# vsahni3/cross-attention-ViT

Measured on AMD Instinct MI355X. Metric: 3D patch-tokens/sec fwd+bwd, 2-modality 128^3 p16 ViT, higher is better.
Workload: dtype bf16; 1 GPU; configs[1]: ModelCross d=768 H=12 mlp=3072 2x2 blocks, 2 modalities, 128^3 volume, 16^3 patches (N=513), dropout 0; per_gpu_batch=126, global_batch=126, seq_len=513, parallelism=dp1, step=zero-grad + weight bf16 cast + fwd + loss + bwd, optimizer_step=excluded, launch=eager (one launch per kernel)

## Files before the change

cross-attention-vit_amd/csrc/gemm.hip:

```cpp
#include "xvit_common.h"

#include <atomic>
#include <mutex>
#include <algorithm>
#include <string>

namespace xvit {

struct GemmParams {
  const bf16* A; const bf16* B; void* C; const float* bias; const float* res; bf16* aux;
  int64_t lda, ldb, ldc, ldr, ldaux;
  int64_t sA, sB, sC, sBias, sR, sAux;
  int M, N, K, k_per_split, split_k, ntm, ntn;
  int c_f32, act, accumulate;
  int res_row_mod, res_row_off, seg_rows, seg_skip, row_off;
  float* slab;
  float* colsum;
  float drop_p, drop_inv; uint64_t drop_seed;
  const uint64_t* drop_epoch;
  int aux_deriv;
  int narrow_epi;
  int ncg;
  struct PatchGather {
    int mode;
// ... 285 lines not shown
      }
    }
  }
  if (csum && !part) {
#pragma unroll
    for (int e = 0; e < 4; ++e) {
      float t = cs4[e];
      t += __shfl_xor(t, 16);
      t += __shfl_xor(t, 32);
      cs4[e] = t;
    }
    if (lane < 16 && col < p.N) {
#pragma unroll
      for (int e = 0; e < 4; ++e) unsafeAtomicAdd(csum + col + e, cs4[e]);
    }
  }
}

constexpr int TBM = 256, TBN = 256;
constexpr int T_OPER = TBM * BK * 2;
constexpr int T_STAGE = 2 * T_OPER;
constexpr int T_LDS = 2 * T_STAGE;

__device__ __forceinline__ int gather_krow_token(const GemmParams::PatchGather& g, int kr) {
  const int nw = 64 / g.Dn;
  if (nw & 1) return kr;
  const int a = kr >> 1, b = kr & 1, wa = a / g.Dn, d = a - wa * g.Dn;
  return d + g.Dn * (2 * wa + b);
}

template <bool KS>
struct BigLoader {
  __amdgpu_buffer_rsrc_t rsrc;
  uint32_t voff[4];
  uint32_t kstep;
  __device__ __forceinline__ void init(const bf16* tile_base, int64_t bytes_avail, int64_t ld, int wave, int lane, const GemmParams::PatchGather* perm = nullptr) {
    rsrc = make_rsrc(tile_base, clamp_bytes(bytes_avail));
#pragma unroll
    for (int j = 0; j < 4; ++j) {
      const int piece = wave * 4 + j;
      if (KS) {
        const int krow = piece * 2 + (lane >> 5);
        const int chunk = (lane & 31) ^ swz_ks(krow);
        const int srow = perm ? gather_krow_token(*perm, krow) : krow;
        voff[j] = (uint32_t)(srow * ld * 2 + chunk * 16);
      } else {
        const int row = piece * 8 + (lane >> 3);
        const int chunk = (lane & 7) ^ swz_kc(row);
        voff[j] = (uint32_t)(row * ld * 2 + chunk * 16);
      }
    }
    kstep = KS ? (uint32_t)(BK * ld * 2) : (uint32_t)(BK * 2);
  }
  __device__ __forceinline__ void init_gather_rows(const GemmParams::PatchGather& g, const bf16* vol, int m0, int M, int wave, int lane) {
    rsrc = make_rsrc(vol, g.vol_bytes);
#pragma unroll
    for (int j = 0; j < 4; ++j) {
      const int ii = lane >> 3, rl = (wave * 4 + j) * 8 + ii, row = m0 + wave * 32 + (ii & 3) * 8 + 2 * j + (ii >> 2);
      const int chunk = (lane & 7) ^ swz_kc(rl);
      const int smp = row / g.ntok, n = row - smp * g.ntok;
      voff[j] = (row < M && n >= g.cls) ? 2u * (gather_sample_origin(g, smp) + gather_patch_origin(g, n - g.cls) + gather_elem_off(g, chunk * 8)) : GATHER_OOB;
    }
    kstep = 0;
  }
  __device__ __forceinline__ void init_gather_ks(const GemmParams::PatchGather& g, const bf16* vol, int n0, int N, int wave, int lane) {
    rsrc = make_rsrc(vol, g.vol_bytes);
#pragma unroll
    for (int j = 0; j < 4; ++j) {
      const int krow = (wave * 4 + j) * 2 + (lane >> 5);
      const int e = n0 + (((lane & 31) ^ swz_ks(krow)) << 3);
      const int tok = gather_krow_token(g, krow);
      voff[j] = e < N ? 2u * ((uint32_t)((tok % g.Dn) * g.dp * g.Sz + (tok / g.Dn) * g.wp) + gather_elem_off(g, e)) : GATHER_OOB;
    }
    kstep = 0;
  }
  __device__ __forceinline__ void place_tokens(const GemmParams::PatchGather& g, int ktg, uint32_t total, int64_t ld, bool volume, const uint32_t (&fixed)[4], int wave, int lane) {
#pragma unroll
    for (int j = 0; j < 4; ++j) {
      const int krow = (wave * 4 + j) * 2 + (lane >> 5);
      const GatherTok t = gather_token(g, (uint32_t)ktg * 64u + (uint32_t)krow, total);
      voff[j] = !t.ok || fixed[j] == GATHER_OOB ? GATHER_OOB : (volume ? 2u * t.vol + fixed[j] : t.row * (uint32_t)(ld * 2) + fixed[j]);
    }
  }
  __device__ __forceinline__ void issue_at(XVIT_LDS char* image, int wave, uint32_t soff) const {
#pragma unroll
    for (int j = 0; j < 4; ++j) glds16(rsrc, image + (wave * 4 + j) * 1024, voff[j], soff);
  }
  __device__ __forceinline__ void issue(XVIT_LDS char* image, int wave, int kt) const { issue_at(image, wave, (uint32_t)kt * kstep); }
};

__device__ __forceinline__ uint32_t gather_soff_rows(const GemmParams::PatchGather& g, int ktg) { return 2u * gather_elem_off(g, ktg * 64); }
struct GatherStep { uint32_t a, b; };
__device__ __forceinline__ GatherStep gather_soff_wgrad(const GemmParams::PatchGather& g, int ktg, int64_t lda) {
  const int spk = g.pcount >> 6, smp = ktg / spk, r = ktg - smp * spk;
  const int wsteps = (g.Dn * g.Wn) >> 6, h = r / wsteps, wpart = (r - h * wsteps) * (64 / g.Dn);
  GatherStep o;
  o.a = (uint32_t)(((int64_t)smp * g.ntok + g.cls + r * 64) * lda * 2);
  o.b = 2u * (gather_sample_origin(g, smp) + (uint32_t)(h * g.hp * g.Sy + wpart * g.wp));
  return o;
}

typedef __attribute__((__vector_size__(4 * sizeof(unsigned)))) unsigned u32x4_dbg;
template <bool KS, int NT_>
struct BigFrag {
  uint32_t off[KS ? 2 * NT_ : 2];
  __device__ __forceinline__ void init(int first, int lane) {
    if (KS) {
      const int g = lane >> 4, i = lane & 15, q = i >> 2, p = i & 3;
#pragma unroll
      for (int t = 0; t < NT_; ++t)
#pragma unroll
        for (int s = 0; s < 2; ++s) {
          const int krow = 8 * g + 4 * s + q;
          const int ch = (first + t) * 2 + (p >> 1);
          off[t * 2 + s] = (uint32_t)(512 * krow + 16 * (ch ^ swz_ks(krow)) + 8 * (p & 1));
        }
    } else {
      const int row = first * 16 + (lane & 15);
#pragma unroll
      for (int kk = 0; kk < 2; ++kk) off[kk] = (uint32_t)(row * 128 + (((kk * 4 + (lane >> 4)) ^ swz_kc(row)) << 4));
    }
  }
  __device__ __forceinline__ bf16x8 read(const XVIT_LDS char* image, int t, int kk) const {
#ifdef XVIT_DEBUG_NO_LDSREAD
    u32x4_dbg v = {off[0] * 2654435761u, off[0] * 40503u + 12345u, (uint32_t)t * 0x9E3779B9u ^ off[0], 0x3F803F80u ^ (off[0] << 3)};
    v &= 0xBFFFBFFFu;
    asm volatile("" : "+v"(v));
    return __builtin_bit_cast(bf16x8, v);
#endif
    if (KS) {
      const s16x4 lo = lds_read_tr16(image + off[t * 2 + 0] + kk * 32 * 512);
      const s16x4 hi = lds_read_tr16(image + off[t * 2 + 1] + kk * 32 * 512);
      s16x8 v = {lo[0], lo[1], lo[2], lo[3], hi[0], hi[1], hi[2], hi[3]};
      return __builtin_bit_cast(bf16x8, v);
    } else {
      return *(const XVIT_LDS bf16x8*)(image + off[kk] + t * 16 * 128);
    }
  }
};

template <int S, int PF, int NA, int NB>
__device__ __forceinline__ void mma_sched_steps() {
  constexpr int reads = (S + PF < 16 ? NA : 0) + (S >= 4 && S < 8 ? NB : 0);
  if constexpr (reads > 0) __builtin_amdgcn_sched_group_barrier(0x100, reads, 0);
  __builtin_amdgcn_sched_group_barrier(0x008, 4, 0);
  if constexpr (S + 1 < 16) mma_sched_steps<S + 1, PF, NA, NB>();
}

template <bool A_KS, bool B_KS>
__device__ __forceinline__ void big_tile_mma(const XVIT_LDS char* sa, const XVIT_LDS char* sb, const BigFrag<A_KS, 8>& fa, const BigFrag<B_KS, 4>& fb,
                                             f32x4 (&acc)[8][4], const BigLoader<A_KS>& la, const BigLoader<B_KS>& lb, __amdgpu_buffer_rsrc_t ra,
                                             __amdgpu_buffer_rsrc_t rb, XVIT_LDS char* nxt, int wave, uint32_t soff_a, uint32_t soff_b) {
  constexpr int PF = 2;
  constexpr int NA = A_KS ? 2 : 1, NB = B_KS ? 2 : 1;
  bf16x8 b0[4], b1[4], a[16];
#pragma unroll
  for (int t = 0; t < 4; ++t) b0[t] = fb.read(sb, t, 0);
#pragma unroll
  for (int s = 0; s < PF; ++s) a[s] = fa.read(sa, s & 7, s >> 3);
#pragma unroll
  for (int s = 0; s < 16; ++s) {
#ifndef XVIT_DEBUG_NO_DMA
    if (s < 4) glds16(ra, nxt + (wave * 4 + s) * 1024, la.voff[s], soff_a);
    else if (s < 8) glds16(rb, nxt + T_OPER + (wave * 4 + s - 4) * 1024, lb.voff[s - 4], soff_b);
#endif
    if (s + PF < 16) a[s + PF] = fa.read(sa, (s + PF) & 7, (s + PF) >> 3);
    if (s >= 4 && s < 8) b1[s - 4] = fb.read(sb, s - 4, 1);
#pragma unroll
    for (int j = 0; j < 4; ++j)
      acc[s & 7][j] = __builtin_amdgcn_mfma_f32_16x16x32_bf16(s < 8 ? b0[j] : b1[j], a[s], acc[s & 7][j], 0, 0, 0);
  }
  __builtin_amdgcn_sched_group_barrier(0x100, 4 * NB + PF * NA, 0);
  mma_sched_steps<0, PF, NA, NB>();
}

#ifndef XVIT_EPI_STORE_AUX
#define XVIT_EPI_STORE_AUX 2
#endif
#ifndef XVIT_EPI_LOAD_AUX
#define XVIT_EPI_LOAD_AUX 2
#endif
#ifndef XVIT_EPI_RES_AUX
#define XVIT_EPI_RES_AUX 2
#endif
typedef __attribute__((__vector_size__(2 * sizeof(unsigned)))) unsigned u32x2_t;
typedef __attribute__((__vector_size__(4 * sizeof(unsigned)))) unsigned u32x4_t;
constexpr uint32_t OOB = 0xFFFFFFF0u;
constexpr int EPI_WAVE_BYTES = 64 * 256;

struct BigEpi {
  __amdgpu_buffer_rsrc_t rc, raux, rres, rslab;
  bool has_res, has_aux, to_slab;
  uint32_t col;
  bool col_ok;
  f32x4 bias;
  f32x4 csum;
  float* colsum_dst;
  uint64_t drop_base;
  uint32_t row, c, aux, res, slab;
  uint32_t rrem, rmod, srem, smod;
  uint32_t c_step, aux_step, res_step, slab_step, c_gap, res_wrap;
};

struct LoadCursor { uint32_t row, aux; };
struct EpiLoads { u32x2_t aux[4]; };

// ... 187 lines not shown
  for (int b = 0; b < 2; ++b) {
    const int it = (R & 3) * 2 + b;
    const f32x4 v0 = *(const XVIT_LDS f32x4*)(slice + it * 2048 + roffw[it & 1][0]);
    const f32x4 v1 = *(const XVIT_LDS f32x4*)(slice + it * 2048 + roffw[it & 1][1]);
    wide_body<ACT, DROP>(p, e, v0, v1, cur.aux[b]);
  }
  __builtin_amdgcn_sched_barrier(0);
  if constexpr (R < 7) wide_regions<ACT, DROP, R + 1>(p, e, lc, nxt, acc, slice, woff, roffw);
}

template <int ACT, bool DROP>
__device__ __forceinline__ void wide_epilogue(const GemmParams& p, WideEpi& e, const f32x4 (&acc)[8][4], XVIT_LDS char* slice, const uint32_t (&woff)[4],
                                              const uint32_t (&roffw)[2][2], float* colsum_dst) {
  WideCursor lc = {e.row, e.aux};
  WideLoads first;
  if constexpr (ACT == XVIT_ACT_DGELU || ACT == ACT_MULAUX) wide_issue_aux(p, e, lc, first);
  wide_regions<ACT, DROP, 0>(p, e, lc, first, acc, slice, woff, roffw);
  if (colsum_dst) {
#pragma unroll
    for (int c = 0; c < 4; ++c) {
      float t0 = e.csum0[c], t1 = e.csum1[c];
#pragma unroll
      for (int o = 8; o < 64; o <<= 1) { t0 += __shfl_xor(t0, o); t1 += __shfl_xor(t1, o); }
      e.csum0[c] = t0; e.csum1[c] = t1;
    }
    if ((threadIdx.x & 63) < 8 && e.col_ok) {
#pragma unroll
      for (int c = 0; c < 4; ++c) { unsafeAtomicAdd(colsum_dst + c, e.csum0[c]); unsafeAtomicAdd(colsum_dst + 4 + c, e.csum1[c]); }
    }
  }
}

template <int ACT>
__device__ __forceinline__ void wave_tile_epilogue_wide(const GemmParams& p, const f32x4 (&acc)[8][4], XVIT_LDS char* smem, int wave, int lane, int row0, int col0,
                                                        int batch) {
  WideEpi e;
  e.rc = make_rsrc((const char*)p.C + batch * p.sC * 2, clamp_bytes(0x7FFFFFF0ll));
  e.has_aux = p.aux != nullptr;
  const bool has_bias = p.bias != nullptr;
  e.raux = make_rsrc(e.has_aux ? (const void*)(p.aux + batch * p.sAux) : (const void*)p.C, e.has_aux ? 0x7FFFFFF0u : 0u);
  const __amdgpu_buffer_rsrc_t rbias = make_rsrc(has_bias ? (const void*)(p.bias + batch * p.sBias) : (const void*)p.C, has_bias ? (uint32_t)(p.N * 4) : 0u);
  int pin = 0;
  asm volatile("" : "+v"(pin));
  const int wl = lane + pin;
  uint32_t woff[4], roffw[2][2];
  {
    const int r = wl & 15, g = wl >> 4, c = wl & 7, rr = wl >> 3;
#pragma unroll
    for (int j = 0; j < 4; ++j) woff[j] = (uint32_t)(r * 256 + (((j * 4 + g) ^ r) << 4));
#pragma unroll
    for (int par = 0; par < 2; ++par)
#pragma unroll
      for (int k = 0; k < 2; ++k) roffw[par][k] = (uint32_t)(rr * 256 + (((2 * c + k) ^ ((par * 8 + rr) & 15)) << 4));
  }
  XVIT_LDS char* slice = smem + wave * EPI_WAVE_BYTES;
  e.col = (uint32_t)(col0 + (wl & 7) * 8);
  e.col_ok = e.col < (uint32_t)p.N;
  e.bias0 = __builtin_bit_cast(f32x4, __builtin_amdgcn_raw_buffer_load_b128(rbias, e.col * 4, 0, 0));
  e.bias1 = __builtin_bit_cast(f32x4, __builtin_amdgcn_raw_buffer_load_b128(rbias, e.col * 4 + 16, 0, 0));
  e.drop_base = (uint64_t)batch * ((uint64_t)p.M * p.N);
  e.csum0 = f32x4{0.f, 0.f, 0.f, 0.f}; e.csum1 = f32x4{0.f, 0.f, 0.f, 0.f};
  float* colsum_dst = p.colsum ? p.colsum + batch * p.sBias + e.col : nullptr;
  e.row = (uint32_t)(row0 + (wl >> 3));
  e.c = e.row * (uint32_t)p.ldc * 2u + e.col * 2u;
  e.aux = e.row * (uint32_t)p.ldaux * 2u + e.col * 2u;
  e.c_step = 8u * (uint32_t)p.ldc * 2u;
  e.aux_step = 8u * (uint32_t)p.ldaux * 2u;
  wide_epilogue<ACT, false>(p, e, acc, slice, woff, roffw, colsum_dst);
}

template <bool PERM = false>
__device__ __forceinline__ void wave_tile_epilogue(const GemmParams& p, const f32x4 (&acc)[8][4], XVIT_LDS char* smem, int wave, int lane, int row0, int col0,
                                                   int batch, int split) {
  const int nbatch = gridDim.z / p.split_k;
  BigEpi e;
  const int64_t celt = p.c_f32 ? 4 : 2;
  e.rc = make_rsrc((const char*)p.C + batch * p.sC * celt, clamp_bytes(0x7FFFFFF0ll));
  e.has_aux = p.aux != nullptr; e.has_res = p.res != nullptr; e.to_slab = p.slab != nullptr;
  const bool has_bias = p.bias != nullptr;
  e.raux = make_rsrc(e.has_aux ? (const void*)(p.aux + batch * p.sAux) : (const void*)p.C, e.has_aux ? 0x7FFFFFF0u : 0u);
  e.rres = make_rsrc(e.has_res ? (const void*)(p.res + batch * p.sR) : (const void*)p.C, e.has_res ? 0x7FFFFFF0u : 0u);
  const __amdgpu_buffer_rsrc_t rbias = make_rsrc(has_bias ? (const void*)(p.bias + batch * p.sBias) : (const void*)p.C, has_bias ? (uint32_t)(p.N * 4) : 0u);
  e.rslab = make_rsrc(e.to_slab ? (const void*)(p.slab + ((int64_t)split * nbatch + batch) * (int64_t)p.M * p.N) : (const void*)p.C,
                      e.to_slab ? clamp_bytes((int64_t)p.M * p.N * 4) : 0u);
  int pin = 0;
  asm volatile("" : "+v"(pin));
  const int wl = lane + pin;
  uint32_t woff[8], roff[4];
  {
    const int r = wl & 15, g = wl >> 4, k = wl & 15, rr = wl >> 4;
#pragma unroll
    for (int j = 0; j < 4; ++j) woff[j] = woff[4 + j] = (uint32_t)(r * 256 + (((j * 4 + g) ^ r) << 4));
    if constexpr (PERM) {
#pragma unroll
      for (int half = 0; half < 2; ++half) {
        const int l32 = 16 * half + r, jj = l32 >> 3, ii = l32 & 7, rho = (ii & 3) * 8 + 2 * jj + (ii >> 2);
#pragma unroll
        for (int j = 0; j < 4; ++j) woff[half * 4 + j] = (uint32_t)(rho * 256 + (((j * 4 + g) ^ (rho & 15)) << 4));
      }
    }
#pragma unroll
    for (int q = 0; q < 4; ++q) roff[q] = (uint32_t)(rr * 256 + ((k ^ (q * 4 + rr)) << 4));
  }
  XVIT_LDS char* slice = smem + wave * EPI_WAVE_BYTES;
  e.col = (uint32_t)(col0 + (wl & 15) * 4);
  e.col_ok = e.col < (uint32_t)p.N;
  e.bias = __builtin_bit_cast(f32x4, __builtin_amdgcn_raw_buffer_load_b128(rbias, e.col * 4, 0, 0));
  e.drop_base = (uint64_t)batch * ((uint64_t)p.M * p.N);
  e.csum = f32x4{0.f, 0.f, 0.f, 0.f};
  e.colsum_dst = p.colsum ? p.colsum + batch * p.sBias + e.col : nullptr;
  e.row = (uint32_t)(row0 + (wl >> 4));
  {
    const bool rmap = p.res_row_mod > 0, smap = p.seg_rows > 0;
    e.rmod = rmap ? (uint32_t)p.res_row_mod : 0x7FFFFFFFu;
    e.smod = smap ? (uint32_t)p.seg_rows : 0x7FFFFFFFu;
    e.rrem = rmap ? e.row % e.rmod : e.row;
    e.srem = smap ? e.row % e.smod : e.row;
    const uint32_t rrow = rmap ? (uint32_t)p.res_row_off + e.rrem : e.row;
    const uint32_t orow = smap ? e.row + (e.row / e.smod) * (uint32_t)p.seg_skip + (uint32_t)p.row_off : e.row;
    const uint32_t ce = p.c_f32 ? 4u : 2u;
    e.c = orow * (uint32_t)p.ldc * ce + e.col * ce;
    e.aux = e.row * (uint32_t)p.ldaux * 2u + e.col * 2u;
    e.res = rrow * (uint32_t)p.ldr * 4u + e.col * 4u;
    e.slab = e.row * (uint32_t)p.N * 4u + e.col * 4u;
    e.c_step = 4u * (uint32_t)p.ldc * ce;
    e.aux_step = 4u * (uint32_t)p.ldaux * 2u;
    e.res_step = 4u * (uint32_t)p.ldr * 4u;
    e.slab_step = 4u * (uint32_t)p.N * 4u;
    e.c_gap = smap ? (uint32_t)p.seg_skip * (uint32_t)p.ldc * ce : 0u;
    e.res_wrap = rmap ? e.rmod * (uint32_t)p.ldr * 4u : 0u;
  }
  if constexpr (PERM) {
    big_epilogue<XVIT_ACT_NONE, false, true>(p, e, acc, slice, woff, roff);
    return;
  }
  if (p.drop_p > 0.f) {
    if (p.act == XVIT_ACT_GELU) big_epilogue<XVIT_ACT_GELU, true>(p, e, acc, slice, woff, roff);
    else if (p.act == XVIT_ACT_DGELU) big_epilogue<XVIT_ACT_DGELU, true>(p, e, acc, slice, woff, roff);
    else big_epilogue<XVIT_ACT_NONE, true>(p, e, acc, slice, woff, roff);
  } else if (p.act == XVIT_ACT_GELU) big_epilogue<XVIT_ACT_GELU, false>(p, e, acc, slice, woff, roff);
  else if (p.act == XVIT_ACT_DGELU) big_epilogue<XVIT_ACT_DGELU, false>(p, e, acc, slice, woff, roff);
  else big_epilogue<XVIT_ACT_NONE, false>(p, e, acc, slice, woff, roff);
}

#ifdef XVIT_GEMM_CLOCK_PROBE
__device__ long long xvit_dbg_clk[2 * 4096];
struct ClockProbe {
  long long c0, w0;
  __device__ ClockProbe() : c0(clock64()), w0(wall_clock64()) {}
  __device__ ~ClockProbe() {
    if (threadIdx.x == 0 && blockIdx.z == 0 && blockIdx.x < 4096) { xvit_dbg_clk[2 * blockIdx.x] = clock64() - c0; xvit_dbg_clk[2 * blockIdx.x + 1] = wall_clock64() - w0; }
  }
};
#endif
template <bool A_KS, bool B_KS, int WIDE_ACT, int GATHER = 0>
__global__ __launch_bounds__(512, 2) void gemm_big_kernel(const GemmParams p) {
  extern __shared__ __attribute__((aligned(16))) char smem_raw[];
  XVIT_LDS char* smem = (XVIT_LDS char*)smem_raw;
#ifdef XVIT_GEMM_CLOCK_PROBE
  ClockProbe clock_probe;
#endif
  const int tid = threadIdx.x, lane = tid & 63, wave = uniform(tid >> 6);
  const int wr = wave >> 2, wc = wave & 3;

  const int nblk = gridDim.x, total = nblk * gridDim.z, lin = blockIdx.x + nblk * blockIdx.z;
  const int q8 = total >> 3, r8 = total & 7, xcd = lin & 7;
  const int logical = (xcd < r8 ? xcd * (q8 + 1) : r8 * (q8 + 1) + (xcd - r8) * q8) + (lin >> 3);
  const int zz = logical / nblk, tile = logical - zz * nblk;
  const int grp = min(tile / (p.ntm * p.ncg), (p.ntn - 1) / p.ncg);
  const int rem = tile - grp * p.ntm * p.ncg;
  const int gw = min(p.ncg, p.ntn - grp * p.ncg);
  const int tm = rem / gw, tn = grp * p.ncg + (rem - tm * gw);
  const int m0 = tm * TBM, n0 = tn * TBN;
  const int batch = zz / p.split_k, split = zz - batch * p.split_k;
  const int k_begin = split * p.k_per_split;
  const int k_end = min(p.K, k_begin + p.k_per_split);
  const int nk = (k_end - k_begin + BK - 1) / BK;

  BigLoader<A_KS> la;
  BigLoader<B_KS> lb;
  {
    const bf16* Ab = p.A + batch * p.sA;
    if constexpr (GATHER == 1) la.init_gather_rows(p.g, Ab, m0, p.M, wave, lane);
    else if constexpr (GATHER == 2 || GATHER == 3) {
      const int64_t rows = (int64_t)(p.K / p.g.pcount) * p.g.ntok;
      la.init(Ab + m0, ((rows - 1) * p.lda + (p.M - m0)) * 2, p.lda, wave, lane, GATHER == 2 ? &p.g : nullptr);
    } else if (A_KS) la.init(Ab + (int64_t)k_begin * p.lda + m0, ((int64_t)(k_end - 1 - k_begin) * p.lda + (p.M - m0)) * 2, p.lda, wave, lane);
    else la.init(Ab + (int64_t)m0 * p.lda + k_begin, ((int64_t)(p.M - 1 - m0) * p.lda + (k_end - k_begin)) * 2, p.lda, wave, lane);
    const bf16* Bb = p.B + batch * p.sB;
    if constexpr (GATHER == 2 || GATHER == 3) lb.init_gather_ks(p.g, Bb, n0, p.N, wave, lane);
    else if (B_KS) lb.init(Bb + (int64_t)k_begin * p.ldb + n0, ((int64_t)(k_end - 1 - k_begin) * p.ldb + (p.N - n0)) * 2, p.ldb, wave, lane);
    else lb.init(Bb + (int64_t)n0 * p.ldb + k_begin, ((int64_t)(p.N - 1 - n0) * p.ldb + (k_end - k_begin)) * 2, p.ldb, wave, lane);
  }
  const int ktg0 = k_begin / BK;
  uint32_t fix_a[4], fix_b[4];
  if constexpr (GATHER == 3) {
#pragma unroll
    for (int j = 0; j < 4; ++j) {
      const int krow = (wave * 4 + j) * 2 + (lane >> 5);
      const int chunk = (lane & 31) ^ swz_ks(krow);
      fix_a[j] = m0 + chunk * 8 < p.M ? (uint32_t)(chunk * 16) : GATHER_OOB;
      const int e = n0 + (chunk << 3);
      fix_b[j] = e < p.N ? 2u * gather_elem_off(p.g, e) : GATHER_OOB;
    }
  }
  auto step_off = [&](int kt, uint32_t& oa, uint32_t& ob) {
    if constexpr (GATHER == 1) { oa = gather_soff_rows(p.g, ktg0 + kt); ob = (uint32_t)kt * lb.kstep; }
    else if constexpr (GATHER == 2) { GatherStep o; o = gather_soff_wgrad(p.g, ktg0 + kt, p.lda); oa = o.a; ob = o.b; }
    else if constexpr (GATHER == 3) {
      la.place_tokens(p.g, ktg0 + kt, (uint32_t)p.K, p.lda, false, fix_a, wave, lane);
      lb.place_tokens(p.g, ktg0 + kt, (uint32_t)p.K, 0, true, fix_b, wave, lane);
      oa = ob = 0u;
    }
    else { oa = (uint32_t)kt * la.kstep; ob = (uint32_t)kt * lb.kstep; }
  };
  BigFrag<A_KS, 8> fa;
  BigFrag<B_KS, 4> fb;
  fa.init(wr * 8, lane);
  fb.init(wc * 4, lane);

  f32x4 acc[8][4];
#pragma unroll
  for (int i = 0; i < 8; ++i)
#pragma unroll
    for (int j = 0; j < 4; ++j) acc[i][j] = f32x4{0.f, 0.f, 0.f, 0.f};

  const __amdgpu_buffer_rsrc_t null_rsrc = make_rsrc(p.A, 0u);
  if (nk > 0) {
    uint32_t oa, ob;
    step_off(0, oa, ob);
    la.issue_at(smem, wave, oa);
    lb.issue_at(smem + T_OPER, wave, ob);
  }
  for (int kt = 0; kt < nk; ++kt) {
    asm volatile("s_waitcnt vmcnt(0)" ::: "memory");
    __syncthreads();
    const bool more = kt + 1 < nk;
    uint32_t soff_a, soff_b;
    step_off(kt + 1, soff_a, soff_b);
    XVIT_LDS char* nxt = smem + ((kt + 1) & 1) * T_STAGE;
    const XVIT_LDS char* sa = smem + (kt & 1) * T_STAGE;
    const XVIT_LDS char* sb = sa + T_OPER;
#ifndef XVIT_DEBUG_NO_MMA
    big_tile_mma<A_KS, B_KS>(sa, sb, fa, fb, acc, la, lb, more ? la.rsrc : null_rsrc, more ? lb.rsrc : null_rsrc, nxt, wave, soff_a, soff_b);
#endif
  }

  asm volatile("s_waitcnt vmcnt(0)" ::: "memory");
  __syncthreads();
  if constexpr (WIDE_ACT >= 0) wave_tile_epilogue_wide<WIDE_ACT>(p, acc, smem, wave, lane, m0 + wr * 128, n0 + wc * 64, batch);
  else wave_tile_epilogue<GATHER == 1>(p, acc, smem, wave, lane, m0 + wr * 128, n0 + wc * 64, batch, split);
}

__global__ void splitk_epilogue_kernel(const GemmParams p, int nbatch) {
  const int nv = p.N >> 2;
  const int64_t per = (int64_t)p.M * nv, total = per * nbatch;
  for (int64_t i = (int64_t)blockIdx.x * blockDim.x + threadIdx.x; i < total; i += (int64_t)gridDim.x * blockDim.x) {
    const int b = (int)(i / per);
    const int64_t r = i - (int64_t)b * per;
    const int row = (int)(r / nv), col = (int)(r - (int64_t)row * nv) * 4;
    f32x4 v = {0.f, 0.f, 0.f, 0.f};
    for (int s = 0; s < p.split_k; ++s) v += *(const f32x4*)(p.slab + (((int64_t)s * nbatch + b) * p.M + row) * p.N + col);
    const f32x4 o = epilogue_apply_rt(p, v, row, col, b * p.sC, p.bias ? p.bias + b * p.sBias : nullptr, p.res ? p.res + b * p.sR : nullptr,
                                      p.aux ? p.aux + b * p.sAux : nullptr);
    if (p.colsum) {
#pragma unroll
      for (int e = 0; e < 4; ++e) unsafeAtomicAdd(p.colsum + b * p.sBias + col + e, o[e]);
    }
  }
}

}

using namespace xvit;

static bool aligned16(const void* p) { return (reinterpret_cast<uintptr_t>(p) & 15) == 0; }

static std::atomic<int> g_gemm_tile{0};
static std::atomic<int> g_gemm_epi{0};
static std::atomic<int> g_gemm_group{0};

static bool use_big_tile(const xvit_gemm_args* a) {
  if (a->M < 256 || a->N < 256 || g_gemm_tile.load(std::memory_order_relaxed) == 1) return false;
  if (g_gemm_tile.load(std::memory_order_relaxed) == 2) return true;
// ... 64 lines not shown
  p.seg_rows = a->out_seg_rows; p.seg_skip = a->out_seg_skip; p.row_off = a->out_row_off;
  p.slab = ws_need > 0 ? (float*)a->workspace : nullptr;
  p.colsum = a->colsum;
  XVIT_REQUIRE(a->dropout_p >= 0.f && a->dropout_p < 1.f, "xvit_gemm: dropout_p must be in [0, 1)");
  p.drop_p = a->dropout_p; p.drop_inv = 1.0f / (1.0f - a->dropout_p); p.drop_seed = a->dropout_seed;
  p.drop_epoch = a->dropout_p > 0.f ? drop_epoch_ptr() : nullptr;
  p.narrow_epi = g_gemm_epi.load(std::memory_order_relaxed);
  p.aux_deriv = a->aux_mode;
  p.ncg = 1;
  p.g.mode = 0;
  hipStream_t s = (hipStream_t)stream;

  static std::once_flag attr_once;
  std::call_once(attr_once, [] {
    (void)hipFuncSetAttribute((const void*)gemm_kernel<false, false>, hipFuncAttributeMaxDynamicSharedMemorySize, GEMM_LDS);
    (void)hipFuncSetAttribute((const void*)gemm_kernel<false, true>, hipFuncAttributeMaxDynamicSharedMemorySize, GEMM_LDS);
    (void)hipFuncSetAttribute((const void*)gemm_kernel<true, true>, hipFuncAttributeMaxDynamicSharedMemorySize, GEMM_LDS);
    (void)hipFuncSetAttribute((const void*)gemm_big_kernel<false, false, -1>, hipFuncAttributeMaxDynamicSharedMemorySize, T_LDS);
    (void)hipFuncSetAttribute((const void*)gemm_big_kernel<false, true, -1>, hipFuncAttributeMaxDynamicSharedMemorySize, T_LDS);
    (void)hipFuncSetAttribute((const void*)gemm_big_kernel<true, true, -1>, hipFuncAttributeMaxDynamicSharedMemorySize, T_LDS);
    (void)hipFuncSetAttribute((const void*)gemm_big_kernel<false, false, XVIT_ACT_NONE>, hipFuncAttributeMaxDynamicSharedMemorySize, T_LDS);
    (void)hipFuncSetAttribute((const void*)gemm_big_kernel<false, false, XVIT_ACT_GELU>, hipFuncAttributeMaxDynamicSharedMemorySize, T_LDS);
    (void)hipFuncSetAttribute((const void*)gemm_big_kernel<false, true, XVIT_ACT_NONE>, hipFuncAttributeMaxDynamicSharedMemorySize, T_LDS);
    (void)hipFuncSetAttribute((const void*)gemm_big_kernel<false, true, XVIT_ACT_DGELU>, hipFuncAttributeMaxDynamicSharedMemorySize, T_LDS);
    (void)hipFuncSetAttribute((const void*)gemm_big_kernel<false, false, ACT_GELU_D>, hipFuncAttributeMaxDynamicSharedMemorySize, T_LDS);
    (void)hipFuncSetAttribute((const void*)gemm_big_kernel<false, true, ACT_MULAUX>, hipFuncAttributeMaxDynamicSharedMemorySize, T_LDS);
  });
  if (big) {
    p.ntm = (a->M + TBM - 1) / TBM; p.ntn = (a->N + TBN - 1) / TBN;
    {
      const int forced = g_gemm_group.load(std::memory_order_relaxed);
      p.ncg = forced > 0 ? std::min(forced, p.ntn) : (a->layout == XVIT_GEMM_NT && p.ntn >= 6 ? 3 : p.ntn);
    }
    const dim3 grid(p.ntm * p.ntn, 1, a->batch * a->split_k), block(512);
    const bool wide = !p.c_f32 && !p.slab && !p.res && p.seg_rows == 0 && !p.narrow_epi && p.drop_p == 0.f && a->layout != XVIT_GEMM_TN &&
                      ((p.N | (int)p.ldc | (int)p.ldaux) & 7) == 0 && (a->layout == XVIT_GEMM_NT ? p.act != XVIT_ACT_DGELU : p.act != XVIT_ACT_GELU);
    if (wide && a->layout == XVIT_GEMM_NT && p.act == XVIT_ACT_NONE) hipLaunchKernelGGL((gemm_big_kernel<false, false, XVIT_ACT_NONE>), grid, block, T_LDS, s, p);
    else if (wide && a->layout == XVIT_GEMM_NT && p.aux_deriv) hipLaunchKernelGGL((gemm_big_kernel<false, false, ACT_GELU_D>), grid, block, T_LDS, s, p);
    else if (wide && a->layout == XVIT_GEMM_NT) hipLaunchKernelGGL((gemm_big_kernel<false, false, XVIT_ACT_GELU>), grid, block, T_LDS, s, p);
    else if (wide && p.act == XVIT_ACT_NONE) hipLaunchKernelGGL((gemm_big_kernel<false, true, XVIT_ACT_NONE>), grid, block, T_LDS, s, p);
    else if (wide && p.aux_deriv) hipLaunchKernelGGL((gemm_big_kernel<false, true, ACT_MULAUX>), grid, block, T_LDS, s, p);
    else if (wide) hipLaunchKernelGGL((gemm_big_kernel<false, true, XVIT_ACT_DGELU>), grid, block, T_LDS, s, p);
    else if (a->layout == XVIT_GEMM_NT) hipLaunchKernelGGL((gemm_big_kernel<false, false, -1>), grid, block, T_LDS, s, p);
    else if (a->layout == XVIT_GEMM_NN) hipLaunchKernelGGL((gemm_big_kernel<false, true, -1>), grid, block, T_LDS, s, p);
    else hipLaunchKernelGGL((gemm_big_kernel<true, true, -1>), grid, block, T_LDS, s, p);
  } else {
    p.ntm = (a->M + BM - 1) / BM; p.ntn = (a->N + BN - 1) / BN;
    const dim3 grid(p.ntm * p.ntn, 1, a->batch * a->split_k), block(256);
    switch (a->layout) {
      case XVIT_GEMM_NT: hipLaunchKernelGGL((gemm_kernel<false, false>), grid, block, GEMM_LDS, s, p); break;
      case XVIT_GEMM_NN: hipLaunchKernelGGL((gemm_kernel<false, true>), grid, block, GEMM_LDS, s, p); break;
      default: hipLaunchKernelGGL((gemm_kernel<true, true>), grid, block, GEMM_LDS, s, p); break;
    }
  }
  if (p.slab) {
    const int64_t work = (int64_t)a->batch * a->M * (a->N / 4);
    const int g = (int)((work + 255) / 256 > 4096 ? 4096 : (work + 255) / 256);
    hipLaunchKernelGGL(splitk_epilogue_kernel, dim3(g), dim3(256), 0, s, p, a->batch);
  }
  return check_launch("xvit_gemm");
}

static int64_t pe_rows(const xvit_patch_geom* g) {
  return (int64_t)g->M * g->B * (g->cls_rows + (int64_t)(g->D / g->dp) * (g->H / g->hp) * (g->W / g->wp));
}

extern "C" int xvit_patch_embed_supported(const xvit_patch_geom* g, int d) {
// ... 34 lines not shown
  p.lda = p.ldb = p.ldc = p.ldr = p.ldaux = 0;
  p.sA = p.sB = p.sC = p.sBias = p.sR = p.sAux = 0;
  p.c_f32 = 1; p.act = XVIT_ACT_NONE; p.accumulate = 0;
  p.res_row_mod = 0; p.res_row_off = 0; p.seg_rows = 0; p.seg_skip = 0; p.row_off = 0;
  p.drop_p = 0.f; p.drop_inv = 1.f; p.drop_seed = 0; p.drop_epoch = nullptr; p.narrow_epi = 1; p.split_k = 1; p.aux_deriv = 0;
}

static void pe_attrs() {
  static std::once_flag once;
  std::call_once(once, [] {
    (void)hipFuncSetAttribute((const void*)gemm_big_kernel<false, false, -1, 1>, hipFuncAttributeMaxDynamicSharedMemorySize, T_LDS);
    (void)hipFuncSetAttribute((const void*)gemm_big_kernel<true, true, -1, 2>, hipFuncAttributeMaxDynamicSharedMemorySize, T_LDS);
    (void)hipFuncSetAttribute((const void*)gemm_big_kernel<true, true, -1, 3>, hipFuncAttributeMaxDynamicSharedMemorySize, T_LDS);
  });
}

extern "C" int xvit_patch_embed_fwd(const void* img, const xvit_patch_geom* g, const void* W, int64_t ldw, const float* bias, const float* pos, int64_t ldpos,
                                    float* x, int64_t ldx, int d, xvit_stream_t stream) {
  XVIT_REQUIRE(img && g && W && x, "xvit_patch_embed_fwd: null pointer");
  XVIT_REQUIRE(xvit_patch_embed_supported(g, d) == 1, "xvit_patch_embed_fwd: geometry not supported by the fused kernel (xvit_patch_embed_supported)");
  const int64_t pd = (int64_t)g->dp * g->hp * g->wp;
  XVIT_REQUIRE(ldw >= pd && ldw % 8 == 0 && ldx >= d && ldx % 4 == 0 && (!pos || (ldpos >= d && ldpos % 4 == 0)), "xvit_patch_embed_fwd: bad leading dimension");
  XVIT_REQUIRE(aligned16(img) && aligned16(W) && aligned16(x) && (!bias || aligned16(bias)) && (!pos || aligned16(pos)), "xvit_patch_embed_fwd: pointers must be 16-byte aligned");
  GemmParams p;
  pe_defaults(p);
  pe_fill(p, g, 1);
  p.A = (const bf16*)img; p.B = (const bf16*)W; p.C = x; p.bias = bias; p.res = pos;
  p.ldb = ldw; p.ldc = ldx; p.ldr = ldpos;
  p.M = (int)pe_rows(g); p.N = d; p.K = (int)pd;
  p.k_per_split = p.K;
  if (pos) { p.res_row_mod = p.g.ntok; p.res_row_off = 0; }
  p.ntm = (p.M + TBM - 1) / TBM; p.ntn = (p.N + TBN - 1) / TBN; p.ncg = p.ntn;
  pe_attrs();
  hipLaunchKernelGGL((gemm_big_kernel<false, false, -1, 1>), dim3(p.ntm * p.ntn, 1, 1), dim3(512), T_LDS, (hipStream_t)stream, p);
  return check_launch("xvit_patch_embed_fwd");
}

static int pe_wgrad_split(const xvit_patch_geom* g, int d) {
  const int64_t pd = (int64_t)g->dp * g->hp * g->wp;
  const int tiles = (int)((d / 256) * (pd / 256));
  const int64_t ksteps = pe_rows(g) / 64;
  int split = 256 / (tiles > 0 ? tiles : 1);
  if (split > ksteps / 8) split = (int)(ksteps / 8);
  if (split > 16) split = 16;
  return split < 1 ? 1 : split;
}

extern "C" int64_t xvit_patch_embed_wgrad_workspace_bytes(const xvit_patch_geom* g, int d) {
  if (!g || xvit_patch_embed_supported(g, d) != 1) return 0;
  const int split = pe_wgrad_split(g, d);
  return split > 1 ? (int64_t)split * d * g->dp * g->hp * g->wp * (int64_t)sizeof(float) : 0;
}

extern "C" int xvit_patch_embed_wgrad(const void* img, const xvit_patch_geom* g, const void* dx, int64_t lddx, float* dW, int64_t lddw, int d, void* workspace,
                                      int64_t workspace_bytes, xvit_stream_t stream) {
  XVIT_REQUIRE(img && g && dx && dW, "xvit_patch_embed_wgrad: null pointer");
  XVIT_REQUIRE(xvit_patch_embed_supported(g, d) == 1, "xvit_patch_embed_wgrad: geometry not supported by the fused kernel (xvit_patch_embed_supported)");
  const int64_t pd = (int64_t)g->dp * g->hp * g->wp;
  XVIT_REQUIRE(lddx >= d && lddx % 8 == 0 && lddw >= pd && lddw % 4 == 0, "xvit_patch_embed_wgrad: bad leading dimension");
  XVIT_REQUIRE(aligned16(img) && aligned16(dx) && aligned16(dW), "xvit_patch_embed_wgrad: pointers must be 16-byte aligned");
  XVIT_REQUIRE(pe_rows(g) * lddx * 2 < (1ll << 31), "xvit_patch_embed_wgrad: dx exceeds 2 GiB (unsupported addressing range)");
  const int64_t need = xvit_patch_embed_wgrad_workspace_bytes(g, d);
  XVIT_REQUIRE(need == 0 || (workspace && workspace_bytes >= need && aligned16(workspace)), "xvit_patch_embed_wgrad: needs %lld bytes of 16-byte aligned workspace (got %lld)",
               (long long)need, (long long)workspace_bytes);
  GemmParams p;
  pe_defaults(p);
  const bool aligned = pe_aligned(g);
  pe_fill(p, g, aligned ? 2 : 3);
  p.A = (const bf16*)dx; p.B = (const bf16*)img; p.C = dW;
  p.lda = lddx; p.ldc = lddw;
  p.M = d; p.N = (int)pd;
  p.K = (int)((int64_t)g->M * g->B * p.g.pcount);
  p.split_k = pe_wgrad_split(g, d);
  const int ktiles = (p.K + BK - 1) / BK;
  p.k_per_split = ((ktiles + p.split_k - 1) / p.split_k) * BK;
  p.slab = need > 0 ? (float*)workspace : nullptr;
  p.ntm = (p.M + TBM - 1) / TBM; p.ntn = (p.N + TBN - 1) / TBN; p.ncg = p.ntn;
  pe_attrs();
  hipStream_t s = (hipStream_t)stream;
  if (aligned) hipLaunchKernelGGL((gemm_big_kernel<true, true, -1, 2>), dim3(p.ntm * p.ntn, 1, p.split_k), dim3(512), T_LDS, s, p);
  else hipLaunchKernelGGL((gemm_big_kernel<true, true, -1, 3>), dim3(p.ntm * p.ntn, 1, p.split_k), dim3(512), T_LDS, s, p);
  if (p.slab) {
    const int64_t work = (int64_t)p.M * (p.N / 4);
    const int gsz = (int)((work + 255) / 256 > 4096 ? 4096 : (work + 255) / 256);
    hipLaunchKernelGGL(splitk_epilogue_kernel, dim3(gsz), dim3(256), 0, s, p, 1);
  }
  return check_launch("xvit_patch_embed_wgrad");
}

#ifdef XVIT_GEMM_CLOCK_PROBE
extern "C" int xvit_dbg_read_clk(long long* out, int n) { return (int)hipMemcpyFromSymbol(out, HIP_SYMBOL(xvit::xvit_dbg_clk), (size_t)n * 16); }
#endif
```

Before: 3.718 million patch-tokens/s.

## Use 4-wave 256x256 GEMM blocks with 128x128 per-wave tiles and AGPR accumulators

Measured after the change: 3.455 million patch-tokens/s, median of 2. 7.1% lower.

```diff
diff --git a/cross-attention-vit_amd/csrc/gemm.hip b/cross-attention-vit_amd/csrc/gemm.hip
--- a/cross-attention-vit_amd/csrc/gemm.hip
+++ b/cross-attention-vit_amd/csrc/gemm.hip
@@ -341,13 +341,13 @@
 template <bool KS>
 struct BigLoader {
   __amdgpu_buffer_rsrc_t rsrc;
-  uint32_t voff[4];
+  uint32_t voff[8];
   uint32_t kstep;
   __device__ __forceinline__ void init(const bf16* tile_base, int64_t bytes_avail, int64_t ld, int wave, int lane, const GemmParams::PatchGather* perm = nullptr) {
     rsrc = make_rsrc(tile_base, clamp_bytes(bytes_avail));
 #pragma unroll
-    for (int j = 0; j < 4; ++j) {
-      const int piece = wave * 4 + j;
+    for (int j = 0; j < 8; ++j) {
+      const int piece = wave * 8 + j;
       if (KS) {
         const int krow = piece * 2 + (lane >> 5);
         const int chunk = (lane & 31) ^ swz_ks(krow);
@@ -364,8 +364,8 @@
   __device__ __forceinline__ void init_gather_rows(const GemmParams::PatchGather& g, const bf16* vol, int m0, int M, int wave, int lane) {
     rsrc = make_rsrc(vol, g.vol_bytes);
 #pragma unroll
-    for (int j = 0; j < 4; ++j) {
-      const int ii = lane >> 3, rl = (wave * 4 + j) * 8 + ii, row = m0 + wave * 32 + (ii & 3) * 8 + 2 * j + (ii >> 2);
+    for (int j = 0; j < 8; ++j) {
+      const int pc = wave * 8 + j, jj = pc & 3, ii = lane >> 3, rl = pc * 8 + ii, row = m0 + (pc >> 2) * 32 + (ii & 3) * 8 + 2 * jj + (ii >> 2);
       const int chunk = (lane & 7) ^ swz_kc(rl);
       const int smp = row / g.ntok, n = row - smp * g.ntok;
       voff[j] = (row < M && n >= g.cls) ? 2u * (gather_sample_origin(g, smp) + gather_patch_origin(g, n - g.cls) + gather_elem_off(g, chunk * 8)) : GATHER_OOB;
@@ -375,25 +375,25 @@
   __device__ __forceinline__ void init_gather_ks(const GemmParams::PatchGather& g, const bf16* vol, int n0, int N, int wave, int lane) {
     rsrc = make_rsrc(vol, g.vol_bytes);
 #pragma unroll
-    for (int j = 0; j < 4; ++j) {
-      const int krow = (wave * 4 + j) * 2 + (lane >> 5);
+    for (int j = 0; j < 8; ++j) {
+      const int krow = (wave * 8 + j) * 2 + (lane >> 5);
       const int e = n0 + (((lane & 31) ^ swz_ks(krow)) << 3);
       const int tok = gather_krow_token(g, krow);
       voff[j] = e < N ? 2u * ((uint32_t)((tok % g.Dn) * g.dp * g.Sz + (tok / g.Dn) * g.wp) + gather_elem_off(g, e)) : GATHER_OOB;
     }
     kstep = 0;
   }
-  __device__ __forceinline__ void place_tokens(const GemmParams::PatchGather& g, int ktg, uint32_t total, int64_t ld, bool volume, const uint32_t (&fixed)[4], int wave, int lane) {
-#pragma unroll
-    for (int j = 0; j < 4; ++j) {
-      const int krow = (wave * 4 + j) * 2 + (lane >> 5);
+  __device__ __forceinline__ void place_tokens(const GemmParams::PatchGather& g, int ktg, uint32_t total, int64_t ld, bool volume, const uint32_t (&fixed)[8], int wave, int lane) {
+#pragma unroll
+    for (int j = 0; j < 8; ++j) {
+      const int krow = (wave * 8 + j) * 2 + (lane >> 5);
       const GatherTok t = gather_token(g, (uint32_t)ktg * 64u + (uint32_t)krow, total);
       voff[j] = !t.ok || fixed[j] == GATHER_OOB ? GATHER_OOB : (volume ? 2u * t.vol + fixed[j] : t.row * (uint32_t)(ld * 2) + fixed[j]);
     }
   }
   __device__ __forceinline__ void issue_at(XVIT_LDS char* image, int wave, uint32_t soff) const {
 #pragma unroll
-    for (int j = 0; j < 4; ++j) glds16(rsrc, image + (wave * 4 + j) * 1024, voff[j], soff);
+    for (int j = 0; j < 8; ++j) glds16(rsrc, image + (wave * 8 + j) * 1024, voff[j], soff);
   }
   __device__ __forceinline__ void issue(XVIT_LDS char* image, int wave, int kt) const { issue_at(image, wave, (uint32_t)kt * kstep); }
 };
@@ -412,18 +412,16 @@
 typedef __attribute__((__vector_size__(4 * sizeof(unsigned)))) unsigned u32x4_dbg;
 template <bool KS, int NT_>
 struct BigFrag {
-  uint32_t off[KS ? 2 * NT_ : 2];
+  uint32_t off[2];
   __device__ __forceinline__ void init(int first, int lane) {
     if (KS) {
       const int g = lane >> 4, i = lane & 15, q = i >> 2, p = i & 3;
 #pragma unroll
-      for (int t = 0; t < NT_; ++t)
-#pragma unroll
-        for (int s = 0; s < 2; ++s) {
-          const int krow = 8 * g + 4 * s + q;
-          const int ch = (first + t) * 2 + (p >> 1);
-          off[t * 2 + s] = (uint32_t)(512 * krow + 16 * (ch ^ swz_ks(krow)) + 8 * (p & 1));
-        }
+      for (int s = 0; s < 2; ++s) {
+        const int krow = 8 * g + 4 * s + q;
+        const int ch = first * 2 + (p >> 1);
+        off[s] = (uint32_t)(512 * krow + 16 * (ch ^ swz_ks(krow)) + 8 * (p & 1));
+      }
     } else {
       const int row = first * 16 + (lane & 15);
 #pragma unroll
@@ -438,8 +436,8 @@
     return __builtin_bit_cast(bf16x8, v);
 #endif
     if (KS) {
-      const s16x4 lo = lds_read_tr16(image + off[t * 2 + 0] + kk * 32 * 512);
-      const s16x4 hi = lds_read_tr16(image + off[t * 2 + 1] + kk * 32 * 512);
+      const s16x4 lo = lds_read_tr16(image + (off[0] ^ (uint32_t)(32 * t)) + kk * 32 * 512);
+      const s16x4 hi = lds_read_tr16(image + (off[1] ^ (uint32_t)(32 * t)) + kk * 32 * 512);
       s16x8 v = {lo[0], lo[1], lo[2], lo[3], hi[0], hi[1], hi[2], hi[3]};
       return __builtin_bit_cast(bf16x8, v);
     } else {
@@ -448,39 +446,57 @@
   }
 };
 
-template <int S, int PF, int NA, int NB>
-__device__ __forceinline__ void mma_sched_steps() {
-  constexpr int reads = (S + PF < 16 ? NA : 0) + (S >= 4 && S < 8 ? NB : 0);
-  if constexpr (reads > 0) __builtin_amdgcn_sched_group_barrier(0x100, reads, 0);
-  __builtin_amdgcn_sched_group_barrier(0x008, 4, 0);
-  if constexpr (S + 1 < 16) mma_sched_steps<S + 1, PF, NA, NB>();
+#ifdef XVIT_DEBUG_NO_LDSREAD
+#define XVIT_MFMA_PAD "s_nop 1\n\t"
+#else
+#define XVIT_MFMA_PAD ""
+#endif
+__device__ __forceinline__ void big_mfma(f32x4& acc, const bf16x8& a, const bf16x8& b) {
+  asm volatile(XVIT_MFMA_PAD "v_mfma_f32_16x16x32_bf16 %0, %1, %2, %0" : "+a"(acc) : "v"(a), "v"(b));
+}
+__device__ __forceinline__ void big_acc_fence(f32x4 (&acc)[2][8][4]) {
+  asm volatile("s_nop 11");
+#pragma unroll
+  for (int h = 0; h < 2; ++h)
+#pragma unroll
+    for (int i = 0; i < 8; ++i)
+#pragma unroll
+      for (int j = 0; j < 4; ++j) asm volatile("" : "+a"(acc[h][i][j]));
 }
 
 template <bool A_KS, bool B_KS>
-__device__ __forceinline__ void big_tile_mma(const XVIT_LDS char* sa, const XVIT_LDS char* sb, const BigFrag<A_KS, 8>& fa, const BigFrag<B_KS, 4>& fb,
-                                             f32x4 (&acc)[8][4], const BigLoader<A_KS>& la, const BigLoader<B_KS>& lb, __amdgpu_buffer_rsrc_t ra,
-                                             __amdgpu_buffer_rsrc_t rb, XVIT_LDS char* nxt, int wave, uint32_t soff_a, uint32_t soff_b) {
+__device__ __forceinline__ void big_tile_mma(const XVIT_LDS char* sa, const XVIT_LDS char* sb, const BigFrag<A_KS, 8>& fa, const BigFrag<B_KS, 8>& fb,
+                                             f32x4 (&acc)[2][8][4], bf16x8 (&b0)[8], bf16x8 (&a01)[2], const BigLoader<A_KS>& la,
+                                             const BigLoader<B_KS>& lb, __amdgpu_buffer_rsrc_t ra, __amdgpu_buffer_rsrc_t rb, XVIT_LDS char* nxt, bool more,
+                                             int wave, uint32_t soff_a, uint32_t soff_b) {
   constexpr int PF = 2;
-  constexpr int NA = A_KS ? 2 : 1, NB = B_KS ? 2 : 1;
-  bf16x8 b0[4], b1[4], a[16];
-#pragma unroll
-  for (int t = 0; t < 4; ++t) b0[t] = fb.read(sb, t, 0);
-#pragma unroll
-  for (int s = 0; s < PF; ++s) a[s] = fa.read(sa, s & 7, s >> 3);
+  bf16x8 b1[8], a[16];
+  a[0] = a01[0];
+  a[1] = a01[1];
 #pragma unroll
   for (int s = 0; s < 16; ++s) {
 #ifndef XVIT_DEBUG_NO_DMA
-    if (s < 4) glds16(ra, nxt + (wave * 4 + s) * 1024, la.voff[s], soff_a);
-    else if (s < 8) glds16(rb, nxt + T_OPER + (wave * 4 + s - 4) * 1024, lb.voff[s - 4], soff_b);
+    if (s < 4) {
+      glds16(ra, nxt + (wave * 8 + 2 * s) * 1024, la.voff[2 * s], soff_a);
+      glds16(ra, nxt + (wave * 8 + 2 * s + 1) * 1024, la.voff[2 * s + 1], soff_a);
+    } else if (s < 8) {
+      glds16(rb, nxt + T_OPER + (wave * 8 + 2 * s - 8) * 1024, lb.voff[2 * s - 8], soff_b);
+      glds16(rb, nxt + T_OPER + (wave * 8 + 2 * s - 7) * 1024, lb.voff[2 * s - 7], soff_b);
+    }
 #endif
+    if (s == 14 && more) {
+      asm volatile("s_waitcnt vmcnt(0)" ::: "memory");
+      __syncthreads();
+#pragma unroll
+      for (int t = 0; t < 8; ++t) b0[t] = fb.read(nxt + T_OPER, t, 0);
+      a01[0] = fa.read(nxt, 0, 0);
+      a01[1] = fa.read(nxt, 1, 0);
+    }
     if (s + PF < 16) a[s + PF] = fa.read(sa, (s + PF) & 7, (s + PF) >> 3);
-    if (s >= 4 && s < 8) b1[s - 4] = fb.read(sb, s - 4, 1);
-#pragma unroll
-    for (int j = 0; j < 4; ++j)
-      acc[s & 7][j] = __builtin_amdgcn_mfma_f32_16x16x32_bf16(s < 8 ? b0[j] : b1[j], a[s], acc[s & 7][j], 0, 0, 0);
-  }
-  __builtin_amdgcn_sched_group_barrier(0x100, 4 * NB + PF * NA, 0);
-  mma_sched_steps<0, PF, NA, NB>();
+    if (s < 8) b1[s] = fb.read(sb, s, 1);
+#pragma unroll
+    for (int j = 0; j < 8; ++j) big_mfma(acc[j >> 2][s & 7][j & 3], s < 8 ? b0[j] : b1[j], a[s]);
+  }
 }
 
 #ifndef XVIT_EPI_STORE_AUX
@@ -734,7 +750,7 @@
 }
 
 template <int ACT>
-__device__ __forceinline__ void wave_tile_epilogue_wide(const GemmParams& p, const f32x4 (&acc)[8][4], XVIT_LDS char* smem, int wave, int lane, int row0, int col0,
+__device__ __forceinline__ void wave_tile_epilogue_wide(const GemmParams& p, const f32x4 (&acc)[8][4], XVIT_LDS char* smem, int slot, int lane, int row0, int col0,
                                                         int batch) {
   WideEpi e;
   e.rc = make_rsrc((const char*)p.C + batch * p.sC * 2, clamp_bytes(0x7FFFFFF0ll));
@@ -755,7 +771,7 @@
 #pragma unroll
       for (int k = 0; k < 2; ++k) roffw[par][k] = (uint32_t)(rr * 256 + (((2 * c + k) ^ ((par * 8 + rr) & 15)) << 4));
   }
-  XVIT_LDS char* slice = smem + wave * EPI_WAVE_BYTES;
+  XVIT_LDS char* slice = smem + slot * EPI_WAVE_BYTES;
   e.col = (uint32_t)(col0 + (wl & 7) * 8);
   e.col_ok = e.col < (uint32_t)p.N;
   e.bias0 = __builtin_bit_cast(f32x4, __builtin_amdgcn_raw_buffer_load_b128(rbias, e.col * 4, 0, 0));
@@ -772,7 +788,7 @@
 }
 
 template <bool PERM = false>
-__device__ __forceinline__ void wave_tile_epilogue(const GemmParams& p, const f32x4 (&acc)[8][4], XVIT_LDS char* smem, int wave, int lane, int row0, int col0,
+__device__ __forceinline__ void wave_tile_epilogue(const GemmParams& p, const f32x4 (&acc)[8][4], XVIT_LDS char* smem, int slot, int lane, int row0, int col0,
                                                    int batch, int split) {
   const int nbatch = gridDim.z / p.split_k;
   BigEpi e;
@@ -804,7 +820,7 @@
 #pragma unroll
     for (int q = 0; q < 4; ++q) roff[q] = (uint32_t)(rr * 256 + ((k ^ (q * 4 + rr)) << 4));
   }
-  XVIT_LDS char* slice = smem + wave * EPI_WAVE_BYTES;
+  XVIT_LDS char* slice = smem + slot * EPI_WAVE_BYTES;
   e.col = (uint32_t)(col0 + (wl & 15) * 4);
   e.col_ok = e.col < (uint32_t)p.N;
   e.bias = __builtin_bit_cast(f32x4, __builtin_amdgcn_raw_buffer_load_b128(rbias, e.col * 4, 0, 0));
@@ -856,14 +872,14 @@
 };
 #endif
 template <bool A_KS, bool B_KS, int WIDE_ACT, int GATHER = 0>
-__global__ __launch_bounds__(512, 2) void gemm_big_kernel(const GemmParams p) {
+__global__ __launch_bounds__(256, 1) void gemm_big_kernel(const GemmParams p) {
   extern __shared__ __attribute__((aligned(16))) char smem_raw[];
   XVIT_LDS char* smem = (XVIT_LDS char*)smem_raw;
 #ifdef XVIT_GEMM_CLOCK_PROBE
   ClockProbe clock_probe;
 #endif
   const int tid = threadIdx.x, lane = tid & 63, wave = uniform(tid >> 6);
-  const int wr = wave >> 2, wc = wave & 3;
+  const int wr = wave >> 1, wc = wave & 1;
 
   const int nblk = gridDim.x, total = nblk * gridDim.z, lin = blockIdx.x + nblk * blockIdx.z;
   const int q8 = total >> 3, r8 = total & 7, xcd = lin & 7;
@@ -895,11 +911,11 @@
     else lb.init(Bb + (int64_t)n0 * p.ldb + k_begin, ((int64_t)(p.N - 1 - n0) * p.ldb + (k_end - k_begin)) * 2, p.ldb, wave, lane);
   }
   const int ktg0 = k_begin / BK;
-  uint32_t fix_a[4], fix_b[4];
+  uint32_t fix_a[8], fix_b[8];
   if constexpr (GATHER == 3) {
 #pragma unroll
-    for (int j = 0; j < 4; ++j) {
-      const int krow = (wave * 4 + j) * 2 + (lane >> 5);
+    for (int j = 0; j < 8; ++j) {
+      const int krow = (wave * 8 + j) * 2 + (lane >> 5);
       const int chunk = (lane & 31) ^ swz_ks(krow);
       fix_a[j] = m0 + chunk * 8 < p.M ? (uint32_t)(chunk * 16) : GATHER_OOB;
       const int e = n0 + (chunk << 3);
@@ -917,26 +933,33 @@
     else { oa = (uint32_t)kt * la.kstep; ob = (uint32_t)kt * lb.kstep; }
   };
   BigFrag<A_KS, 8> fa;
-  BigFrag<B_KS, 4> fb;
+  BigFrag<B_KS, 8> fb;
   fa.init(wr * 8, lane);
-  fb.init(wc * 4, lane);
-
-  f32x4 acc[8][4];
-#pragma unroll
-  for (int i = 0; i < 8; ++i)
-#pragma unroll
-    for (int j = 0; j < 4; ++j) acc[i][j] = f32x4{0.f, 0.f, 0.f, 0.f};
+  fb.init(wc * 8, lane);
+
+  f32x4 acc[2][8][4];
+#pragma unroll
+  for (int h = 0; h < 2; ++h)
+#pragma unroll
+    for (int i = 0; i < 8; ++i)
+#pragma unroll
+      for (int j = 0; j < 4; ++j) acc[h][i][j] = f32x4{0.f, 0.f, 0.f, 0.f};
 
   const __amdgpu_buffer_rsrc_t null_rsrc = make_rsrc(p.A, 0u);
+  bf16x8 b0[8], a01[2];
   if (nk > 0) {
     uint32_t oa, ob;
     step_off(0, oa, ob);
     la.issue_at(smem, wave, oa);
     lb.issue_at(smem + T_OPER, wave, ob);
-  }
-  for (int kt = 0; kt < nk; ++kt) {
     asm volatile("s_waitcnt vmcnt(0)" ::: "memory");
     __syncthreads();
+#pragma unroll
+    for (int t = 0; t < 8; ++t) b0[t] = fb.read(smem + T_OPER, t, 0);
+    a01[0] = fa.read(smem, 0, 0);
+    a01[1] = fa.read(smem, 1, 0);
+  }
+  for (int kt = 0; kt < nk; ++kt) {
     const bool more = kt + 1 < nk;
     uint32_t soff_a, soff_b;
     step_off(kt + 1, soff_a, soff_b);
@@ -944,14 +967,25 @@
     const XVIT_LDS char* sa = smem + (kt & 1) * T_STAGE;
     const XVIT_LDS char* sb = sa + T_OPER;
 #ifndef XVIT_DEBUG_NO_MMA
-    big_tile_mma<A_KS, B_KS>(sa, sb, fa, fb, acc, la, lb, more ? la.rsrc : null_rsrc, more ? lb.rsrc : null_rsrc, nxt, wave, soff_a, soff_b);
+    big_tile_mma<A_KS, B_KS>(sa, sb, fa, fb, acc, b0, a01, la, lb, more ? la.rsrc : null_rsrc, more ? lb.rsrc : null_rsrc, nxt, more, wave, soff_a, soff_b);
+#else
+    asm volatile("s_waitcnt vmcnt(0)" ::: "memory");
+    __syncthreads();
 #endif
   }
+  big_acc_fence(acc);
 
   asm volatile("s_waitcnt vmcnt(0)" ::: "memory");
   __syncthreads();
-  if constexpr (WIDE_ACT >= 0) wave_tile_epilogue_wide<WIDE_ACT>(p, acc, smem, wave, lane, m0 + wr * 128, n0 + wc * 64, batch);
-  else wave_tile_epilogue<GATHER == 1>(p, acc, smem, wave, lane, m0 + wr * 128, n0 + wc * 64, batch, split);
+#pragma unroll 1
+  for (int h = 0; h < 2; ++h) {
+    if constexpr (WIDE_ACT >= 0) wave_tile_epilogue_wide<WIDE_ACT>(p, acc[0], smem, 2 * wave + h, lane, m0 + wr * 128, n0 + wc * 128 + h * 64, batch);
+    else wave_tile_epilogue<GATHER == 1>(p, acc[0], smem, 2 * wave + h, lane, m0 + wr * 128, n0 + wc * 128 + h * 64, batch, split);
+#pragma unroll
+    for (int i = 0; i < 8; ++i)
+#pragma unroll
+      for (int j = 0; j < 4; ++j) acc[0][i][j] = acc[1][i][j];
+  }
 }
 
 __global__ void splitk_epilogue_kernel(const GemmParams p, int nbatch) {
@@ -1082,7 +1116,7 @@
       const int forced = g_gemm_group.load(std::memory_order_relaxed);
       p.ncg = forced > 0 ? std::min(forced, p.ntn) : (a->layout == XVIT_GEMM_NT && p.ntn >= 6 ? 3 : p.ntn);
     }
-    const dim3 grid(p.ntm * p.ntn, 1, a->batch * a->split_k), block(512);
+    const dim3 grid(p.ntm * p.ntn, 1, a->batch * a->split_k), block(256);
     const bool wide = !p.c_f32 && !p.slab && !p.res && p.seg_rows == 0 && !p.narrow_epi && p.drop_p == 0.f && a->layout != XVIT_GEMM_TN &&
                       ((p.N | (int)p.ldc | (int)p.ldaux) & 7) == 0 && (a->layout == XVIT_GEMM_NT ? p.act != XVIT_ACT_DGELU : p.act != XVIT_ACT_GELU);
     if (wide && a->layout == XVIT_GEMM_NT && p.act == XVIT_ACT_NONE) hipLaunchKernelGGL((gemm_big_kernel<false, false, XVIT_ACT_NONE>), grid, block, T_LDS, s, p);
@@ -1183,7 +1217,7 @@
   if (pos) { p.res_row_mod = p.g.ntok; p.res_row_off = 0; }
   p.ntm = (p.M + TBM - 1) / TBM; p.ntn = (p.N + TBN - 1) / TBN; p.ncg = p.ntn;
   pe_attrs();
-  hipLaunchKernelGGL((gemm_big_kernel<false, false, -1, 1>), dim3(p.ntm * p.ntn, 1, 1), dim3(512), T_LDS, (hipStream_t)stream, p);
+  hipLaunchKernelGGL((gemm_big_kernel<false, false, -1, 1>), dim3(p.ntm * p.ntn, 1, 1), dim3(256), T_LDS, (hipStream_t)stream, p);
   return check_launch("xvit_patch_embed_fwd");
 }
 
@@ -1229,8 +1263,8 @@
   p.ntm = (p.M + TBM - 1) / TBM; p.ntn = (p.N + TBN - 1) / TBN; p.ncg = p.ntn;
   pe_attrs();
   hipStream_t s = (hipStream_t)stream;
-  if (aligned) hipLaunchKernelGGL((gemm_big_kernel<true, true, -1, 2>), dim3(p.ntm * p.ntn, 1, p.split_k), dim3(512), T_LDS, s, p);
-  else hipLaunchKernelGGL((gemm_big_kernel<true, true, -1, 3>), dim3(p.ntm * p.ntn, 1, p.split_k), dim3(512), T_LDS, s, p);
+  if (aligned) hipLaunchKernelGGL((gemm_big_kernel<true, true, -1, 2>), dim3(p.ntm * p.ntn, 1, p.split_k), dim3(256), T_LDS, s, p);
+  else hipLaunchKernelGGL((gemm_big_kernel<true, true, -1, 3>), dim3(p.ntm * p.ntn, 1, p.split_k), dim3(256), T_LDS, s, p);
   if (p.slab) {
     const int64_t work = (int64_t)p.M * (p.N / 4);
     const int gsz = (int)((work + 255) / 256 > 4096 ? 4096 : (work + 255) / 256);
```
